# simonkosina/vbt

Measured on AMD Instinct MI355X. Metric: frames/sec end-to-end (detect+NMS+track), EfficientDet-Lite0 320x320, higher is better.
Workload: dtype int8

## Files before the change

vbt_amd/csrc/band_block.h:

```cpp
#pragma once
#include <type_traits>

#ifndef VBT_BD_WAVES
#define VBT_BD_WAVES 16
#endif
constexpr int BD_WAVES = VBT_BD_WAVES, BD_THREADS = 64 * BD_WAVES;
constexpr int BD_LIT = 3;
constexpr int BD_LIT_NODE = 1;
constexpr int BD_LIT_NODE_WIDE = 3;
constexpr int BD_WP_TAIL = 1024;

#ifdef VBT_BD_PROF
#define BD_STAMP(k) do { if (threadIdx.x == 0) a.prof[(long)blockIdx.x * 8 + (k)] = __builtin_amdgcn_s_memtime(); } while (0)
#else
#define BD_STAMP(k) do { } while (0)
#endif

struct BandArgs {
  const int8_t* x;
  int8_t* out;
  int H, W, Cout, rows, nbands;
  int C, CS;
  int NCG, KS;
  unsigned zx4;
  const v4i* wd;
  const int* bd;
  const float* md;
  Rq rqd;
  const v4i* wp;
  const int* bp;
  const float* mp;
  Rq rqp;
  int n_src, chain;
  const int8_t* src[3];
  int sh[3], sw[3], smode[3], spt[3], spl[3];
  AddQ sumq, preq;
#ifdef VBT_BD_PROF
  unsigned long long* prof;
#endif
};

__device__ __forceinline__ unsigned band_source4(const BandArgs& a, int j, long b, int iy, int ix, int cd, bool up2) {
  const int C = a.C;
  const int8_t* sb = a.src[j] + b * (long)a.sh[j] * a.sw[j] * C + 4 * cd;
  if (a.smode[j] == 0) return *(const unsigned*)(sb + (iy * a.sw[j] + ix) * C);
  if (a.smode[j] == 1) {
    int yy, xx;
    if (up2) { yy = iy >> 1; xx = ix >> 1; }
    else { yy = (iy * a.sh[j]) / a.H; xx = (ix * a.sw[j]) / a.W; }
    return *(const unsigned*)(sb + (yy * a.sw[j] + xx) * C);
  }
  unsigned lo = 0u, hi = 0u;
#pragma unroll
  for (int ky = 0; ky < 3; ky++) {
    const int yy = iy * 2 + ky - a.spt[j], yc = min(max(yy, 0), a.sh[j] - 1);
#pragma unroll
    for (int kx = 0; kx < 3; kx++) {
      const int xx = ix * 2 + kx - a.spl[j], xc = min(max(xx, 0), a.sw[j] - 1);
      unsigned t = *(const unsigned*)(sb + (yc * a.sw[j] + xc) * C);
      t = (yy == yc && xx == xc) ? (t ^ 0x80808080u) : 0u;
      lo = pk_max_u16(lo, t & 0x00FF00FFu);
      hi = pk_max_u16(hi, (t >> 8) & 0x00FF00FFu);
// ... 4 lines not shown

__device__ __forceinline__ uint4 band_source16(const BandArgs& a, int j, long b, int iy, int ix, int sg, bool up2) {
  const int C = a.C;
  const int8_t* sb = a.src[j] + b * (long)a.sh[j] * a.sw[j] * C + 16 * sg;
  if (a.smode[j] == 0) return *(const uint4*)(sb + (iy * a.sw[j] + ix) * C);
  if (a.smode[j] == 1) {
    int yy, xx;
    if (up2) { yy = iy >> 1; xx = ix >> 1; }
    else { yy = (iy * a.sh[j]) / a.H; xx = (ix * a.sw[j]) / a.W; }
    return *(const uint4*)(sb + (yy * a.sw[j] + xx) * C);
  }
  unsigned lo[4] = {0u, 0u, 0u, 0u}, hi[4] = {0u, 0u, 0u, 0u};
#pragma unroll
  for (int ky = 0; ky < 3; ky++) {
    const int yy = iy * 2 + ky - a.spt[j], yc = min(max(yy, 0), a.sh[j] - 1);
#pragma unroll
    for (int kx = 0; kx < 3; kx++) {
      const int xx = ix * 2 + kx - a.spl[j], xc = min(max(xx, 0), a.sw[j] - 1);
      const uint4 t4 = *(const uint4*)(sb + (yc * a.sw[j] + xc) * C);
      const bool in = yy == yc && xx == xc;
      const unsigned tt[4] = {t4.x, t4.y, t4.z, t4.w};
#pragma unroll
      for (int d = 0; d < 4; d++) {
        const unsigned t = in ? (tt[d] ^ 0x80808080u) : 0u;
        lo[d] = pk_max_u16(lo[d], t & 0x00FF00FFu);
        hi[d] = pk_max_u16(hi[d], (t >> 8) & 0x00FF00FFu);
      }
    }
  }
  return make_uint4((lo[0] | (hi[0] << 8)) ^ 0x80808080u, (lo[1] | (hi[1] << 8)) ^ 0x80808080u, (lo[2] | (hi[2] << 8)) ^ 0x80808080u,
                    (lo[3] | (hi[3] << 8)) ^ 0x80808080u);
}

template <int NW, int CT, bool NODES = true>
__device__ __forceinline__ void sepconv_band_body(const BandArgs& a, int local, unsigned char* bd_smem) {
  constexpr int nwaves = NW, nthreads = 64 * NW;
  constexpr bool C64 = CT == 64, CK = CT != 0;
  constexpr int CS_T = CT == 64 ? 80 : CT;
  static_assert(CT == 0 || CT == 64 || CT == 112, "compile-time widths: 64, 112");
  const long b = fdiv_small(local, frcp(a.nbands));
  const int band = local - (int)b * a.nbands;
  const int tid = threadIdx.x, wave = tid >> 6, lane = tid & 63, r = lane & 15, g = lane >> 4;
  const int y0 = band * a.rows, nr = min(a.rows, a.H - y0);
  const int PW = a.W + 2, NPh = (nr + 2) * PW, NPo = nr * a.W, NPG = (NPo + 15) >> 4;
  const int C = CK ? CT : a.C, CS = CK ? CS_T : a.CS;
  unsigned char* T0 = bd_smem;
  unsigned char* D = T0 + (a.rows + 2) * PW * CS;
  unsigned char* WP = D + (((a.rows * a.W + 15) >> 4) << 4) * CS;
  const int NT = (a.Cout + 15) >> 4, KS = CK ? (CT + 63) / 64 : a.KS, NCG = CK ? (CT + 15) / 16 : a.NCG;
  unsigned char* WB = WP + NT * KS * 1024;
  BD_STAMP(0);

  for (int i = tid; i < NT * KS * 64; i += nthreads) *(v4i*)(WP + 16 * i) = a.wp[i];
  if (tid < 4 * NT) *(uint4*)(WB + 16 * tid) = *(const uint4*)((const unsigned char*)a.bp + 16 * tid);
  else if (tid >= 32 && tid < 32 + 4 * NT) *(uint4*)(WB + 512 + 16 * (tid - 32)) = *(const uint4*)((const unsigned char*)a.mp + 16 * (tid - 32));
  const float rcp_pw = frcp(PW);
  if (NODES && a.n_src > 0) {
    const bool up2[3] = {a.H == 2 * a.sh[0] && a.W == 2 * a.sw[0], a.H == 2 * a.sh[1] && a.W == 2 * a.sw[1], a.H == 2 * a.sh[2] && a.W == 2 * a.sw[2]};
    if (CK || (C & 15) == 0) {
      constexpr int LITN = C64 ? BD_LIT_NODE : BD_LIT_NODE_WIDE;
      const int npp = C64 ? 4 : CS >> 4, nreal = C64 ? 4 : C >> 4;
      const float rcp_npp = frcp(npp);
      const int total = NPh * npp;
      for (int i0 = tid; i0 < total; i0 += LITN * nthreads) {
        uint4 us[LITN][3];
        int pofs[LITN];
#pragma unroll
        for (int k = 0; k < LITN; k++) {
          const int i = i0 + k * nthreads, ic = min(i, total - 1);
          const int p = C64 ? ic >> 2 : (CK ? ic / (CS_T >> 4) : fdiv_small(ic, rcp_npp)), sg = ic - p * npp;
          const int hy = fdiv_small(p, rcp_pw), hx = p - hy * PW;
          const int iy = y0 + hy - 1, ix = hx - 1;
          const bool in = i < total && sg < nreal && iy >= 0 && iy < a.H && ix >= 0 && ix < a.W;
          pofs[k] = i < total ? (p * CS + 16 * sg) | (in ? 0 : (1 << 30)) : -1;
#pragma unroll
          for (int j = 0; j < 3; j++) {
            us[k][j] = make_uint4(0u, 0u, 0u, 0u);
            if (j < a.n_src && in) us[k][j] = band_source16(a, j, b, iy, ix, sg, up2[j]);
          }
        }
#pragma unroll
        for (int k = 0; k < LITN; k++) {
          if (pofs[k] < 0) continue;
          uint4 v = make_uint4(a.zx4, a.zx4, a.zx4, a.zx4);
          if (!(pofs[k] >> 30)) {
            const unsigned u0[4] = {us[k][0].x, us[k][0].y, us[k][0].z, us[k][0].w}, u1[4] = {us[k][1].x, us[k][1].y, us[k][1].z, us[k][1].w},
// ... 64 lines not shown
      const int total = NPh * npp;
      for (int i0 = tid; i0 < total; i0 += BD_LIT * nthreads) {
        uint4 v[BD_LIT];
        int pofs[BD_LIT];
#pragma unroll
        for (int k = 0; k < BD_LIT; k++) {
          const int i = i0 + k * nthreads, ic = min(i, total - 1);
          const int p = CK ? ic / (CS_T >> 4) : fdiv_small(ic, rcp_npp), sg = ic - p * npp;
          const int hy = fdiv_small(p, rcp_pw), hx = p - hy * PW;
          const int iy = y0 + hy - 1, ix = hx - 1;
          pofs[k] = i < total ? p * CS + 16 * sg : -1;
          v[k] = z4;
          if (i < total && sg < nreal && iy >= 0 && iy < a.H && ix >= 0 && ix < a.W) v[k] = *(const uint4*)(xb + (iy * a.W + ix) * C + 16 * sg);
        }
#pragma unroll
        for (int k = 0; k < BD_LIT; k++)
          if (pofs[k] >= 0) *(uint4*)(T0 + pofs[k]) = v[k];
      }
    } else {
    const int ngp = CS >> 3, ng = C >> 3;
    const float rcp_ngp = frcp(ngp);
    const uint2 z2 = make_uint2(a.zx4, a.zx4);
    for (int i = tid; i < NPh * ngp; i += nthreads) {
      const int p = fdiv_small(i, rcp_ngp), sg = i - p * ngp;
      const int hy = fdiv_small(p, rcp_pw), hx = p - hy * PW;
      const int iy = y0 + hy - 1, ix = hx - 1;
      uint2 v = z2;
      if (sg < ng && iy >= 0 && iy < a.H && ix >= 0 && ix < a.W) v = *(const uint2*)(xb + (iy * a.W + ix) * C + 8 * sg);
      *(uint2*)(T0 + p * CS + 8 * sg) = v;
    }
    }
    }
  }
  const int cg = wave % NCG, sub = wave / NCG, nsub = nwaves / NCG;
  v4i wdv[3];
#pragma unroll
  for (int m = 0; m < 3; m++) wdv[m] = a.wd[(cg * 3 + m) * 64 + lane];
  const int4 bq = *(const int4*)(a.bd + 16 * cg + 4 * g);
  const float4 mu = *(const float4*)(a.md + 16 * cg + 4 * g);
  int tapoff[3];
#pragma unroll
  for (int m = 0; m < 3; m++) {
    const int tap = min(4 * m + g, 8);
    tapoff[m] = ((tap / 3) * PW + (tap % 3)) * CS;
  }
  const float rcp_w = frcp(a.W);
  __syncthreads();
  BD_STAMP(1);
  if (sub < nsub) {
    auto d_units = [&](auto full_c, auto u_c, int pg0) {
      constexpr int U = decltype(u_c)::value, FULL = decltype(full_c)::value;
      const unsigned char* pb[U];
      int slot[U];
#pragma unroll
      for (int u = 0; u < U; u++) {
        slot[u] = (pg0 + u * nsub) * 16 + r;
        const int sc = min(slot[u], NPo - 1);
        const int py = fdiv_small(sc, rcp_w);
        pb[u] = T0 + (sc + 2 * py) * CS + 16 * cg;
      }
      v4i bv[U][3], acc[U];
#pragma unroll
      for (int u = 0; u < U; u++)
#pragma unroll
        for (int m = 0; m < 3; m++) bv[u][m] = *(const v4i*)(pb[u] + tapoff[m]);
#pragma unroll
      for (int u = 0; u < U; u++) acc[u] = v4i_from(int4_plus(bq, FULL >= 2 ? RQ_KBIAS : 0));
#pragma unroll
      for (int m = 0; m < 3; m++)
#pragma unroll
        for (int u = 0; u < U; u++) acc[u] = __builtin_amdgcn_mfma_i32_16x16x64_i8(wdv[m], bv[u][m], acc[u], 0, 0, 0);
#pragma unroll
      for (int u = 0; u < U; u++) *(unsigned*)(D + slot[u] * CS + 16 * cg + 4 * g) = rq_pack_b<FULL>(acc[u], mu, a.rqd);
    };
    auto d_walk = [&](auto full_c) {
      int pg = sub;
      for (; pg + nsub < NPG; pg += 2 * nsub) d_units(full_c, std::integral_constant<int, 2>{}, pg);
      if (pg < NPG) d_units(full_c, std::integral_constant<int, 1>{}, pg);
    };
// ... 85 lines not shown
}

#ifndef VBT_BD_HEAD_WAVES
#define VBT_BD_HEAD_WAVES 8
#endif
#ifndef VBT_BD_HEAD_MAXPX
#define VBT_BD_HEAD_MAXPX 240
#endif
constexpr int BD_HEAD_WAVES = VBT_BD_HEAD_WAVES, BD_HEAD_MAXPX = VBT_BD_HEAD_MAXPX;
constexpr int BD_HEAD_WAVES_WIDE = 16;
#ifdef VBT_DEFINE_BAND_KERNELS
__device__ __forceinline__ int band_problem(const MultiTiles& mt) {
  int pi = 0;
#pragma unroll
  for (int i = 1; i < 12; i++)
    if (i < mt.n && (int)blockIdx.x >= mt.start[i]) pi = i;
  return pi;
}
__global__ __launch_bounds__(64 * BD_HEAD_WAVES) void sepconv_band_kernel(const BandArgs* __restrict__ probs, MultiTiles mt) {
  extern __shared__ __attribute__((aligned(16))) unsigned char bd_smem_dyn[];
  const int pi = band_problem(mt);
  sepconv_band_body<BD_HEAD_WAVES, 64, false>(probs[pi], (int)blockIdx.x - mt.start[pi], bd_smem_dyn);
}
__global__ __launch_bounds__(64 * BD_HEAD_WAVES_WIDE, 2) void sepconv_band_wide_kernel(const BandArgs* __restrict__ probs, MultiTiles mt) {
  extern __shared__ __attribute__((aligned(16))) unsigned char bd_smem_dyn[];
  const int pi = band_problem(mt);
  sepconv_band_body<BD_HEAD_WAVES_WIDE, 0, false>(probs[pi], (int)blockIdx.x - mt.start[pi], bd_smem_dyn);
}
__global__ __launch_bounds__(64 * BD_HEAD_WAVES_WIDE, 2) void sepconv_band_c112_kernel(const BandArgs* __restrict__ probs, MultiTiles mt) {
  extern __shared__ __attribute__((aligned(16))) unsigned char bd_smem_dyn[];
  const int pi = band_problem(mt);
  sepconv_band_body<BD_HEAD_WAVES_WIDE, 112, false>(probs[pi], (int)blockIdx.x - mt.start[pi], bd_smem_dyn);
}
__global__ __launch_bounds__(BD_THREADS) void sepconv_band_one_kernel(BandArgs a) {
  extern __shared__ __attribute__((aligned(16))) unsigned char bd_smem_dyn[];
  sepconv_band_body<BD_WAVES, 64>(a, (int)blockIdx.x, bd_smem_dyn);
}
__global__ __launch_bounds__(BD_THREADS) void sepconv_band_one_wide_kernel(BandArgs a) {
  extern __shared__ __attribute__((aligned(16))) unsigned char bd_smem_dyn[];
  sepconv_band_body<BD_WAVES, 0>(a, (int)blockIdx.x, bd_smem_dyn);
}
__global__ __launch_bounds__(BD_THREADS) void sepconv_band_one_c112_kernel(BandArgs a) {
  extern __shared__ __attribute__((aligned(16))) unsigned char bd_smem_dyn[];
  sepconv_band_body<BD_WAVES, 112>(a, (int)blockIdx.x, bd_smem_dyn);
}
#endif
```

vbt_amd/csrc/detector.hip:

```cpp
#include <algorithm>
#include <cmath>
#include <chrono>
#include <functional>
#include <map>
#include <set>
#include <type_traits>
#include <tuple>

#include "launchers.h"

namespace vbt {

static thread_local char g_err[512] = "";
void set_error(const char* fmt, ...) {
  va_list ap;
  va_start(ap, fmt);
  vsnprintf(g_err, sizeof(g_err), fmt, ap);
  va_end(ap);
}

bool lds_opt_in(const void* fn, LdsOptIn* state) {
  int dev = 0;
  if (hipGetDevice(&dev) != hipSuccess || dev < 0 || dev >= 64) { set_error("lds_opt_in: no current HIP device"); return false; }
  if (state->dev[dev] > 0) return true;
// ... 376 lines not shown
  if (xd_force != -100 && (xd_force < 100 || (s.xd2_ok && (xd_force < 200 ? s.xd2_gpw > 0 : s.xd2_gpw16 > 0)))) variant = std::min(xd_force, xd_force / 100 * 100 + s.xd.nchunks);
  ExpDwLaunch L;
  if (s.xd2_ok && (variant >= 100 || variant < 0)) {
    if (variant >= 200 && s.xd2_gpw16 == 0) { L.refuse(VBT_ERR_ARG, "expand + depthwise: plan asks for the 16-wave form on a step that does not support it"); return L; }
    if (variant >= 100 && variant < 200 && s.xd2_gpw == 0) { L.refuse(VBT_ERR_ARG, "expand + depthwise: plan asks for the 8-wave form on a step that does not support it"); return L; }
    const ExpDw2Args& a = s.xd2;
    L.second = true;
    L.nw = (variant >= 200 || (variant < 0 && s.xd2_gpw16 > 0)) ? 16 : 8;
    L.gpw = L.nw == 16 ? s.xd2_gpw16 : s.xd2_gpw;
    L.cpw = std::min(variant >= 100 ? variant % 100 : std::max(1, (a.nchunks * a.nbands * B + 1023) / 1024), a.nchunks);
    L.grid = (unsigned)(B * ((a.nchunks + L.cpw - 1) / L.cpw) * a.nbands);
    L.lds = s.xd2_lds;
    return L;
  }
  if (variant >= 100) { L.refuse(VBT_ERR_ARG, "expand + depthwise: plan asks for the second kernel form on a step that does not support it"); return L; }
  const ExpDwArgs& a = s.xd;
  L.cpw = variant > 0 ? variant : std::max(1, (a.nchunks * a.nbands * B + 511) / 512);
  L.grid = (unsigned)(B * ((a.nchunks + L.cpw - 1) / L.cpw) * a.nbands);
  L.lds = s.lds_bytes;
  return L;
}
static int launch_expdw_step(const vbt_model* m, const Step& s, int B, hipStream_t st, const int8_t* x, int8_t* out) {
  const ExpDwLaunch L = resolve_expdw(m, s, s.variant, B);
  if (L.rc) return L.report();
  const OpRec& dop = m->ops[s.d_op];
  if (L.second) {
    ExpDw2Args a = s.xd2;
    a.x = x; a.out = out; a.cpw = L.cpw;
    return launch_expdw2(a, dop.k, dop.stride, (a.Cin + 63) / 64, L.nw, L.gpw, L.grid, L.lds, st);
  }
  ExpDwArgs a = s.xd;
  a.x = x; a.out = out; a.cpw = L.cpw;
  return launch_expdw(a, dop.k, dop.stride, (a.Cin + 63) / 64, L.grid, L.lds, st);
}

static int launch_step(vbt_model* m, const Step& s, int B, hipStream_t st, const uint8_t* frames, float* boxes, float* scores,
                       float* classes, int* counts, int boff = 0) {
  if (m->pool_dirty) { const int rc = flush_uploads(m); if (rc) return rc; }
  const OpRec& op = m->ops[s.op];
  const TensorRec& to = m->tensors[op.output];
  auto TP = [&](int t) { return m->tptr[t] + (size_t)boff * m->telems[t]; };
  const uint8_t* frame0 = frames;
  int8_t* out = TP(op.output);
  auto member_tiles = [&](auto tiles_of) {
    MultiTiles mt;
    mt.n = (int)s.members.size();
    mt.start[0] = 0;
    for (int i = 0; i < mt.n; i++) mt.start[i + 1] = mt.start[i] + B * tiles_of(s.members[i]);
    return mt;
  };
  const Epi e{s.bias, s.mult, to.zero_point, op.act_min, op.act_max, make_rq(to.zero_point, op.act_min, op.act_max)};
  switch (s.family) {
    case F_STEM: {
      const TensorRec& ti = m->tensors[op.inputs[0]];
      long M = (long)B * to.h * to.w;
      dim3 grid((unsigned)((M + 63) / 64));
      stem_kernel<<<grid, 256, 0, st>>>(frame0, s.wp, e, out, M, ti.h, ti.w, to.h, to.w, to.c, op.pad_t, op.pad_l, ti.zero_point);
      return VBT_OK;
    }
    case F_PW: {
      if (s.members.empty())
        return launch_pw_step(m, s, B, st, TP(m->ops[s.res_op >= 0 ? s.p_op : s.op].inputs[0]),
                              s.res_op >= 0 ? TP(m->ops[s.res_op].inputs[1]) : nullptr, out);
      if (boff != 0) { set_error("merged pointwise convs: sub-batch streams are not supported (VBT_SUBSTREAMS)"); return VBT_ERR_ARG; }
      PwMulti pm;
      memset(&pm, 0, sizeof(pm));
// ... 44 lines not shown
    }
    case F_RESIZE: {
      const TensorRec& ti = m->tensors[op.inputs[0]];
      long total = (long)B * to.h * to.w * (to.c / 4);
      resize_kernel<<<dim3((unsigned)((total + 255) / 256)), 256, 0, st>>>(TP(op.inputs[0]), out, total, ti.h, ti.w, ti.c,
                                                                            to.h, to.w);
      return VBT_OK;
    }
    case F_MULTI: {
      if (boff != 0) {
        for (const Step& ms : s.members) {
          Step t = ms;
          t.variant = s.variant;
          const int rc = launch_step(m, t, B, st, frames, boxes, scores, classes, counts, boff);
          if (rc) return rc;
        }
        return VBT_OK;
      }
      const MultiTiles mt = member_tiles([](const Step& ms) { return ms.fa.tiles_x * ms.fa.tiles_y; });
      const OpRec& dop = m->ops[s.d_op];
      return launch_fused_multi(s.d_multi, mt, dop.k, dop.stride, s.nbp, s.variant != 0, s.lds_bytes, (unsigned)mt.start[mt.n], st);
    }
    case F_MBCONV:
    case F_NODE:
    case F_SEPCONV: {
      FusedArgs a = s.fa;
      a.x = s.e_op >= 0 ? TP(m->ops[s.e_op].inputs[0]) : TP(m->ops[s.d_op].inputs[0]);
      for (int j = 0; j < 3; j++) a.src[j] = s.src_tensor[j] >= 0 ? TP(s.src_tensor[j]) : nullptr;
      a.out = out;
      return launch_fused_step(m, s, a, B, st);
    }
    case F_BAND: {
      if (boff != 0) { set_error("fused_sepconv_band: sub-batch streams are not supported (VBT_SUBSTREAMS)"); return VBT_ERR_ARG; }
      if (s.members.empty()) return launch_band_one(s.bd_args, (unsigned)(B * s.band_tiles), s.lds_bytes, st);
      const MultiTiles mt = member_tiles([](const Step& ms) { return ms.band_tiles; });
      return launch_band_multi(s.d_band, mt, s.members[0].bd_args.C, (unsigned)mt.start[mt.n], s.lds_bytes, st);
    }
    case F_EXPDW:
      return launch_expdw_step(m, s, B, st, TP(m->ops[s.e_op].inputs[0]), out);
    case F_STEMBLK: {
      StemBlockArgs a = s.sb;
      a.frames = frame0;
      a.out = out;
      return launch_stem_block(a, a.rqs.full && a.rqd.full && a.rqp.full, (unsigned)((long)B * a.tiles_x * a.tiles_y), st);
    }
    case F_POST: {
      PostArgs p;
      int base = 0;
      p.C = m->hdr.num_classes > 0 ? m->hdr.num_classes : 1;
      for (int l = 0; l < 5; l++) {
        const TensorRec& tc = m->tensors[op.inputs[l]];
        p.cls[l] = TP(op.inputs[l]);
        p.box[l] = TP(op.inputs[5 + l]);
        p.base[l] = base;
        base += tc.h * tc.w * tc.c / p.C;
      }
      p.base[5] = base;
      p.anchors = m->d_anchors;
      p.tables = m->d_luts;
      p.A = m->hdr.num_anchors;
      p.max_det = m->hdr.max_detections;
      p.iou_thr = m->hdr.nms_iou_threshold;
      int qmin = 128;
      for (int q = 127; q >= -128; q--)
        if (m->post_tables_host[q + 128] >= m->hdr.nms_score_threshold) qmin = q; else break;
      p.qmin = qmin;
      const int lds = post_lds_bytes(p.A);
      if (lds > 64 * 1024) VBT_LDS_OPT_IN(postprocess_kernel);
      if (lds > 160 * 1024 || p.A > 65535) { set_error("decode + NMS: %d anchors do not fit the kernel (LDS %d bytes, 16-bit anchor index)", p.A, lds); return VBT_ERR_CAPACITY; }
// ... 17 lines not shown
  hipEvent_t e0, e1;
  if (hipEventCreate(&e0) != hipSuccess || hipEventCreate(&e1) != hipSuccess) return 1e30;
  float ms = 1e30f;
  int rc = VBT_OK;
  if (nconc <= 1) {
    rc = launch_step(m, s, B, nullptr, m->frames_stage, m->out_boxes, m->out_scores, m->out_classes, m->out_counts);
    (void)hipEventRecord(e0, nullptr);
    for (int r = 0; r < reps && !rc; r++)
      rc = launch_step(m, s, B, nullptr, m->frames_stage, m->out_boxes, m->out_scores, m->out_classes, m->out_counts);
    (void)hipEventRecord(e1, nullptr);
    if (hipEventSynchronize(e1) != hipSuccess || hipEventElapsedTime(&ms, e0, e1) != hipSuccess) ms = 1e30f;
    ms /= reps;
  } else {
    (void)hipDeviceSynchronize();
    for (int i = 0; i < nconc && !rc; i++)
      rc = launch_step(m, s, B, cs[i], m->frames_stage, m->out_boxes, m->out_scores, m->out_classes, m->out_counts);
    (void)hipDeviceSynchronize();
    auto t0 = std::chrono::steady_clock::now();
    for (int r = 0; r < reps; r++)
      for (int i = 0; i < nconc && !rc; i++)
        rc = launch_step(m, s, B, cs[i], m->frames_stage, m->out_boxes, m->out_scores, m->out_classes, m->out_counts);
    (void)hipDeviceSynchronize();
    ms = (float)(std::chrono::duration<double, std::milli>(std::chrono::steady_clock::now() - t0).count() / (reps * nconc));
  }
  (void)hipEventDestroy(e0);
  (void)hipEventDestroy(e1);
  return rc ? 1e30 : ms;
}

static bool is_fused_tile(int family) { return family == F_MBCONV || family == F_SEPCONV || family == F_NODE; }
static bool variant_ok(const vbt_model* m, const Step& st, int v) {
  if (st.family == F_PW) return !st.members.empty() || !resolve_pw(m, st, v, m->max_batch).rc;
  if (is_fused_tile(st.family)) return !resolve_fused(m, st, v, m->max_batch).rc;
  return st.family != F_EXPDW || !resolve_expdw(m, st, v, m->max_batch).rc;
}

static std::vector<int> candidate_variants(const vbt_model* m, const Step& st) {
  std::vector<int> cand{-1};
  const OpRec& op = m->ops[st.op];
  if (st.family == F_DW) {
    cand = {0};
    for (int r : {1, 2, 4, 8, 16})
      if (r <= m->tensors[op.output].h) cand.push_back(r);
    if (m->tensors[op.output].c % 8 == 0) { cand.push_back(100); cand.push_back(101); }
  } else if (st.family == F_PW && st.KS64 <= 4) {
    cand = {0, 1};
  } else if (st.family == F_PW) {
    cand = {-1, 2, 3, 4, 5, 6};
  } else if (is_fused_tile(st.family)) {
    cand = {0, 1, 3, 5};
    if (st.family == F_MBCONV && st.fa.nch3 > 0 && st.nbp <= 2 && st.fa.KSe >= 1 && st.fa.KSe <= 4) { cand.push_back(9); cand.push_back(11); }
    if (st.family == F_MBCONV && st.nbp <= 2 && (st.fa.KSe == 1 || st.fa.KSe == 2)) {
      cand.push_back(17);
      if (st.fa.nch3 > 0) cand.push_back(25);
    }
  } else if (st.family == F_MULTI) {
    cand = {0, 1};
  } else if (st.family == F_EXPDW) {
    cand.clear();
    for (int cpw : {1, 2, 3, 4, 6})
      if (cpw <= st.xd.nchunks) cand.push_back(cpw);
    if (st.xd2_ok)
      for (int cpw : {1, 2, 3, 4, 6})
        if (cpw <= st.xd.nchunks) {
          if (st.xd2_gpw > 0) cand.push_back(100 + cpw);
          if (st.xd2_gpw16 > 0) cand.push_back(200 + cpw);
        }
  }
  cand.erase(std::remove_if(cand.begin(), cand.end(), [&](int v) { return !variant_ok(m, st, v); }), cand.end());
  return cand;
}

static void autotune(vbt_model* m) {
  const int B = (m->max_batch + m->n_sub - 1) / m->n_sub, reps = 4;
  for (Group& g : m->groups) {
    bool single = g.alts.size() == 1 && g.alts[0].steps.size() == 1;
    if (single) {
      int f = g.alts[0].steps[0].family;
      if (f != F_DW && f != F_PW) continue;
    }
    for (Alt& a : g.alts) {
      a.ms = 0;
      for (Step& st : a.steps) {
        const std::vector<int> cand = candidate_variants(m, st);
        double best = 1e30;
        int bestv = -1;
        for (int v : cand) {
          Step t = st;
          t.variant = v;
          double ms = time_step(m, t, B, reps);
          if (getenv("VBT_AUTOTUNE_VERBOSE") && cand.size() > 1 && atoi(getenv("VBT_AUTOTUNE_VERBOSE")) > 1)
            fprintf(stderr, "[autotune]   op %d %s v%d %.1fus\n", st.op, kFamilyName[st.family], v, ms * 1e3);
          if (ms < best) { best = ms; bestv = v; }
        }
        st.variant = bestv;
        st.tuned_ms = best;
        a.ms += best;
      }
    }
    int bi = 0;
// ... 675 lines not shown
```

vbt_amd/csrc/k_band.hip:

```cpp
#define VBT_DEFINE_BAND_KERNELS 1
#include "launchers.h"

namespace vbt {

static int band_attrs() {
  VBT_LDS_OPT_IN(sepconv_band_kernel);
  VBT_LDS_OPT_IN(sepconv_band_one_kernel);
  VBT_LDS_OPT_IN(sepconv_band_wide_kernel);
  VBT_LDS_OPT_IN(sepconv_band_one_wide_kernel);
  VBT_LDS_OPT_IN(sepconv_band_c112_kernel);
  VBT_LDS_OPT_IN(sepconv_band_one_c112_kernel);
  return VBT_OK;
}

int launch_band_one(const BandArgs& a, unsigned grid, int lds_bytes, hipStream_t st) {
  if (band_attrs()) return VBT_ERR_HIP;
  static const bool generic = getenv("VBT_BAND_GENERIC") != nullptr;
  if (a.C == 64) sepconv_band_one_kernel<<<dim3(grid), BD_THREADS, lds_bytes, st>>>(a);
  else if (a.C == 112 && a.CS == 112 && !generic) sepconv_band_one_c112_kernel<<<dim3(grid), BD_THREADS, lds_bytes, st>>>(a);
  else sepconv_band_one_wide_kernel<<<dim3(grid), BD_THREADS, lds_bytes, st>>>(a);
  return VBT_OK;
}

int launch_band_multi(const BandArgs* d_probs, const MultiTiles& mt, int C, unsigned grid, int lds_bytes, hipStream_t st) {
  if (band_attrs()) return VBT_ERR_HIP;
  static const bool generic = getenv("VBT_BAND_GENERIC") != nullptr;
  if (C == 64) sepconv_band_kernel<<<dim3(grid), 64 * BD_HEAD_WAVES, lds_bytes, st>>>(d_probs, mt);
  else if (C == 112 && !generic) sepconv_band_c112_kernel<<<dim3(grid), 64 * BD_HEAD_WAVES_WIDE, lds_bytes, st>>>(d_probs, mt);
  else sepconv_band_wide_kernel<<<dim3(grid), 64 * BD_HEAD_WAVES_WIDE, lds_bytes, st>>>(d_probs, mt);
  return VBT_OK;
}

int launch_expdw(const ExpDwArgs& a, int k, int stride, int KS64, unsigned grid_x, int lds_bytes, hipStream_t st) {
  const dim3 grid(grid_x);
#define XD_LAUNCH(KK, S)                                                                                             \
  do {                                                                                                               \
    VBT_LDS_OPT_IN(expdw_image_kernel<KK, S, 2>);                                                                    \
    VBT_LDS_OPT_IN(expdw_image_kernel<KK, S, 3>);                                                                    \
    VBT_LDS_OPT_IN(expdw_image_kernel<KK, S, 4>);                                                                    \
    if (KS64 == 2) expdw_image_kernel<KK, S, 2><<<grid, XD_THREADS, lds_bytes, st>>>(a);                             \
    else if (KS64 == 3) expdw_image_kernel<KK, S, 3><<<grid, XD_THREADS, lds_bytes, st>>>(a);                        \
    else expdw_image_kernel<KK, S, 4><<<grid, XD_THREADS, lds_bytes, st>>>(a);                                       \
  } while (0)
  if (k == 3 && stride == 1) XD_LAUNCH(3, 1);
  else if (k == 5 && stride == 1) XD_LAUNCH(5, 1);
  else XD_LAUNCH(5, 2);
#undef XD_LAUNCH
  return VBT_OK;
}

template <int KK, int S, int KS64, int NW, int GPW>
static int launch_expdw2_t(const ExpDw2Args& a, unsigned grid, int lds_bytes, hipStream_t st) {
  VBT_LDS_OPT_IN(expdw2_kernel<KK, S, KS64, NW, GPW>);
  expdw2_kernel<KK, S, KS64, NW, GPW><<<dim3(grid), 64 * NW, lds_bytes, st>>>(a);
  return VBT_OK;
}

int launch_expdw2(const ExpDw2Args& a, int k, int stride, int KS64, int nw, int gpw, unsigned grid, int lds_bytes, hipStream_t st) {
#define XD2_GPW(KK, KS)                                                                    \
  do {                                                                                     \
// ... 41 lines not shown
```

vbt_amd/csrc/launchers.h:

```cpp
#pragma once
#include "dev_common.h"

namespace vbt {
#include "fused_block.h"
#include "stem_block.h"
#include "image_block.h"
#include "expdw_block.h"
#include "expdw2_block.h"
#include "band_block.h"

struct FusedLaunch {
  int k, stride, nbp;
  bool expand;
  bool mdw;
  bool nt3;
  bool ppw2;
  bool dw64;
  int lds_bytes;
  unsigned grid;
};
int launch_fused_block(const FusedArgs& a, const FusedLaunch& L, hipStream_t st);
int launch_fused_multi(const FusedArgs* d_args, const MultiTiles& mt, int k, int stride, int nbp, bool mdw, int lds_bytes, unsigned grid,
                       hipStream_t st);
int launch_dw_tile(const DwTileArgs& a, int k, int stride, bool mdw, dim3 grid, int lds_bytes, hipStream_t st);
int launch_mbconv_image(const FusedArgs& a, const ImageBundle& wb, int k, int stride, int maxu, int PW, int PH, int NB, int lds_bytes, int B,
                        hipStream_t st);
int launch_band_one(const BandArgs& a, unsigned grid, int lds_bytes, hipStream_t st);
int launch_band_multi(const BandArgs* d_probs, const MultiTiles& mt, int C, unsigned grid, int lds_bytes, hipStream_t st);
int launch_expdw(const ExpDwArgs& a, int k, int stride, int KS64, unsigned grid, int lds_bytes, hipStream_t st);
int launch_expdw2(const ExpDw2Args& a, int k, int stride, int KS64, int nw, int gpw, unsigned grid, int lds_bytes, hipStream_t st);
int launch_stem_block(const StemBlockArgs& a, bool full_range, unsigned grid, hipStream_t st);

}
```

vbt_amd/csrc/planner.h:

```cpp
#pragma once

static int conv_kb(const vbt_model* m, const OpRec& op) {
  const bool off = getenv("VBT_NO_KBIAS") != nullptr;
  if (off || (op.type != OP_STEM && op.type != OP_PW && op.type != OP_DW)) return 0;
  const TensorRec& tin = m->tensors[op.inputs[0]];
  const TensorRec& tout = m->tensors[op.output];
  const int8_t* w = (const int8_t*)(m->blob.data() + op.w_off);
  const int32_t* bq = (const int32_t*)(m->blob.data() + op.b_off);
  const bool dw = op.type == OP_DW;
  const int N = tout.c, K = dw ? op.k * op.k : op.k * op.k * tin.c;
  for (int co = 0; co < N; co++) {
    long long sa = 0;
    for (int k = 0; k < K; k++) sa += std::abs((int)(dw ? w[(size_t)k * N + co] : w[(size_t)co * K + k]));
    if (255 * sa + std::llabs((long long)bq[co]) >= (1ll << 22) - 1) return 0;
  }
  return 1;
}

static void choose_tile(int OH, int OW, int KK, int S, bool expand, int* TXo, int* TYo, int slots = 64) {
  double best = 1e300;
  for (int TX = 1; TX <= std::min(OW, 64); TX++) {
    int TXp = (TX + 3) & ~3;
    int TY = std::min(OH, slots / TXp);
    if (TY < 1) continue;
// ... 162 lines not shown
    std::vector<v4i> wp3;
    pack_weights64(wpj, tout.c, Ce, nch3, s.nbp, wp3, &kmap);
    long *d1, *d2;
    v4i* d3;
    if ((rc = upload(m, pack_expand48(we, Ce, tin.c, a.KSe), &d1)) || (rc = upload(m, pack_dw_diag(wd, Ce, kk, 48), &d2)) || (rc = upload(m, wp3, &d3))) return rc;
    a.we3 = d1; a.wdm3 = d2; a.wp3 = d3; a.nch3 = nch3; a.KSp3 = nch3;
  }
  if (expand && tin.h * tin.w <= 400 && tout.h * tout.w <= 400 && (rc = make_image_bundle(m, e_op, d_op, p_op, a.KSe, &s.ib))) return rc;
  *out = s;
  return VBT_OK;
}

static const Alt* tile_alt(const Group& g, int family) {
  for (int i = (int)g.alts.size() - 1; i >= 0; i--)
    if (g.alts[i].steps.size() == 1 && g.alts[i].steps[0].family == family) return &g.alts[i];
  return nullptr;
}
static const Alt* band_alt(const Group& g) {
  for (int i = (int)g.alts.size() - 1; i >= 0; i--)
    if (g.alts[i].steps.size() == 1 && g.alts[i].steps[0].family == F_BAND && g.alts[i].steps[0].members.empty()) return &g.alts[i];
  return nullptr;
}

static bool band_ok(const vbt_model* m, int d_op, int p_op) {
  if (m->flags & VBT_MODEL_NO_BAND) return false;
  if (const char* ns = getenv("VBT_SUBSTREAMS")) if (atoi(ns) > 1) return false;
  const OpRec& d = m->ops[d_op];
  const OpRec& p = m->ops[p_op];
  const TensorRec& ti = m->tensors[d.inputs[0]];
  const TensorRec& to = m->tensors[p.output];
  return d.k == 3 && d.stride == 1 && d.pad_t == 1 && d.pad_l == 1 && ti.c % 8 == 0 && ti.c >= 16 && ti.c <= 128 && to.c <= 128 && to.h == ti.h &&
         to.w == ti.w && ti.w <= 160;
}
static int band_lds(const BandArgs& a) {
  const int NT = (a.Cout + 15) / 16;
  return (a.rows + 2) * (a.W + 2) * a.CS + (((a.rows * a.W + 15) >> 4) << 4) * a.CS + NT * a.KS * 1024 + BD_WP_TAIL;
}
static int make_band(vbt_model* m, int d_op, int p_op, int sum_op, const NodeSrc* ns, Step* out) {
  const OpRec& dop = m->ops[d_op];
  const OpRec& pop = m->ops[p_op];
  const TensorRec& tin = m->tensors[dop.inputs[0]];
  const TensorRec& td = m->tensors[dop.output];
  const TensorRec& to = m->tensors[pop.output];
  Step s;
  s.family = F_BAND;
  s.op = p_op;
  s.d_op = d_op;
  s.p_op = p_op;
  s.sum_op = sum_op;
  BandArgs& a = s.bd_args;
  memset(&a, 0, sizeof(a));
  a.H = tin.h; a.W = tin.w; a.Cout = to.c;
  const int C = tin.c;
  a.C = C;
  a.CS = ((C + 15) / 16 | 1) * 16;
  a.NCG = (C + 15) / 16;
  a.KS = (C + 63) / 64;
  static const int band_px_env = getenv("VBT_BAND_PX") ? atoi(getenv("VBT_BAND_PX")) : 0;
  const int band_px = band_px_env > 0 ? band_px_env : (m->max_batch <= 8 ? 64 : 320);
  const int nb = std::max(1, (tin.h * tin.w + band_px - 1) / band_px);
  a.rows = (tin.h + nb - 1) / nb;
  a.nbands = (tin.h + a.rows - 1) / a.rows;
  a.zx4 = (unsigned)(tin.zero_point & 255) * 0x01010101u;
  const int8_t* wd = (const int8_t*)(m->blob.data() + dop.w_off);
  v4i *dpd, *dpp;
  int* dbd;
  float* dmd;
  int rc;
  if ((rc = upload(m, pack_band_dw(wd, C), &dpd)) || (rc = upload(m, pack_band_pw((const int8_t*)(m->blob.data() + pop.w_off), to.c, C), &dpp)) ||
      (rc = upload(m, fold_bias((const int32_t*)(m->blob.data() + dop.b_off), wd, C, 9, tin.zero_point, W_TAPS, a.NCG * 16), &dbd)) ||
      (rc = upload(m, pad_floats((const float*)(m->blob.data() + dop.m_off), C, a.NCG * 16), &dmd)))
    return rc;
  a.wd = dpd; a.wp = dpp; a.bd = dbd; a.md = dmd;
  a.bp = m->op_steps[p_op].bias;
  a.mp = m->op_steps[p_op].mult;
  a.rqd = make_rq(td.zero_point, dop.act_min, dop.act_max, conv_kb(m, dop));
  a.rqp = make_rq(to.zero_point, pop.act_min, pop.act_max, conv_kb(m, pop));
  a.x = m->tptr[dop.inputs[0]];
  a.out = m->tptr[pop.output];
  if (sum_op >= 0) {
    fill_node_sources(a, *ns, m, sum_op);
    a.x = nullptr;
    for (int j = 0; j < ns->n; j++) a.src[j] = m->tptr[ns->tensor[j]];
  }
  s.band_tiles = a.nbands;
  s.lds_bytes = band_lds(a);
  std::vector<BandArgs> one{a};
  if ((rc = upload(m, one, &s.d_band))) return rc;
  s.cost = cost_of(m, {d_op, p_op, sum_op}, ns);
  *out = s;
  return VBT_OK;
}

static int batch_heads(vbt_model* m) {
  struct Info { int gi, chain, depth; };
  std::vector<Info> heads;
  std::map<int, std::pair<int, int>> by_tensor;
  int nchains = 0, first = -1;
  for (int gi = 0; gi < (int)m->groups.size(); gi++) {
    const Group& g = m->groups[gi];
    const Alt* fap = tile_alt(g, F_SEPCONV);
    if (!fap) continue;
    const Step& st = fap->steps[0];
    if (m->ops[st.d_op].level < 0) continue;
    int tin = m->ops[st.d_op].inputs[0], tout = m->ops[st.p_op].output;
    auto it = by_tensor.find(tin);
// ... 848 lines not shown
```

vbt_amd/csrc/weight_pack.h:

```cpp
#pragma once

static void pack_weights(const int8_t* w, int N, int K, int KS, int NB, const std::vector<int>* kmap, std::vector<long>& out) {
  out.assign((size_t)NB * KS * 4 * 64, 0);
  int8_t* o = (int8_t*)out.data();
  for (int nb = 0; nb < NB; nb++)
    for (int ks = 0; ks < KS; ks++)
      for (int t = 0; t < 4; t++)
        for (int lane = 0; lane < 64; lane++) {
          int i = lane & 15, g = lane >> 4;
          int co = 64 * nb + 16 * (i >> 2) + 4 * t + (i & 3);
          for (int j = 0; j < 8; j++) {
            int kp = 32 * ks + 8 * g + j;
            int k = kmap ? (kp < (int)kmap->size() ? (*kmap)[kp] : -1) : (kp < K ? kp : -1);
            int8_t v = (co < N && k >= 0) ? w[(size_t)co * K + k] : 0;
            o[((((size_t)(nb * KS + ks) * 4 + t) * 64 + lane) * 8) + j] = v;
          }
        }
}

static void pack_weights64(const int8_t* w, int N, int K, int KS, int NB, std::vector<v4i>& out, const std::vector<int>* kmap = nullptr) {
  out.assign((size_t)NB * KS * 4 * 64, (v4i){0, 0, 0, 0});
  int8_t* o = (int8_t*)out.data();
  for (int nb = 0; nb < NB; nb++)
    for (int ks = 0; ks < KS; ks++)
// ... 95 lines not shown
  std::vector<int> kmap((size_t)(Ce / 48) * 64, -1);
  for (int c = 0; c < Ce / 48; c++)
    for (int q = 0; q < 48; q++) kmap[(size_t)c * 64 + q] = 48 * c + q;
  return kmap;
}

static std::vector<v4i> pack_band_dw(const int8_t* w, int C) {
  const int NCG = (C + 15) / 16;
  std::vector<v4i> out((size_t)NCG * 3 * 64, (v4i){0, 0, 0, 0});
  int8_t* o = (int8_t*)out.data();
  for (int cg = 0; cg < NCG; cg++)
    for (int mi = 0; mi < 3; mi++)
      for (int lane = 0; lane < 64; lane++) {
        const int i = lane & 15, g = lane >> 4, ch = 16 * cg + i, tap = 4 * mi + g;
        for (int j = 0; j < 16; j++) o[(((size_t)(cg * 3 + mi) * 64 + lane) * 16) + j] = (tap < 9 && j == i && ch < C) ? w[(size_t)tap * C + ch] : 0;
      }
  return out;
}
static std::vector<v4i> pack_band_pw(const int8_t* w, int N, int C) {
  const int NT = (N + 15) / 16, KS = (C + 63) / 64;
  std::vector<v4i> out((size_t)NT * KS * 64, (v4i){0, 0, 0, 0});
  int8_t* o = (int8_t*)out.data();
  for (int t = 0; t < NT; t++)
    for (int ks = 0; ks < KS; ks++)
      for (int lane = 0; lane < 64; lane++) {
        const int i = lane & 15, g = lane >> 4, co = 16 * t + i;
        for (int j = 0; j < 16; j++) {
          const int k = 64 * ks + 16 * g + j;
          o[((((size_t)t * KS + ks) * 64 + lane) * 16) + j] = (co < N && k < C) ? w[(size_t)co * C + k] : 0;
        }
      }
  return out;
}

static std::vector<int> stem_kmap() {
  std::vector<int> kmap(32, -1);
  for (int g = 0; g < 3; g++)
    for (int j = 0; j < 8; j++) kmap[8 * g + j] = (g * 3 + j / 3) * 3 + j % 3;
  for (int j = 0; j < 3; j++) kmap[24 + j] = (j * 3 + 2) * 3 + 2;
  return kmap;
}
static std::vector<long> pack_stem_block_stem(const int8_t* w) {
  std::vector<long> out(2 * 64, 0);
  int8_t* o = (int8_t*)out.data();
  for (int t = 0; t < 2; t++)
    for (int lane = 0; lane < 64; lane++) {
      const int i = lane & 15, kg = lane >> 4, co = 8 * (i >> 2) + 4 * t + (i & 3);
      for (int j = 0; j < 8; j++) {
        const int f = kg < 3 ? kg * 9 + j : (j < 3 ? j * 9 + 8 : -1);
        o[((size_t)t * 64 + lane) * 8 + j] = f >= 0 ? w[(size_t)co * 27 + f] : 0;
      }
    }
  return out;
}
static std::vector<long> pack_stem_block_proj(const int8_t* w, int N) {
  std::vector<long> out(64, 0);
  int8_t* o = (int8_t*)out.data();
  for (int lane = 0; lane < 64; lane++) {
    const int i = lane & 15, kg = lane >> 4;
    for (int j = 0; j < 8; j++) o[(size_t)lane * 8 + j] = i < N ? w[(size_t)i * 32 + 8 * kg + j] : 0;
  }
  return out;
}

static std::vector<v4i> pack_expdw_expand(const int8_t* w, int Ce, int K) {
  const int nch = (Ce + 63) / 64, KS = (K + 63) / 64;
// ... 46 lines not shown
```

Before: 115,700.

## Add chained depthwise-to-pointwise band kernel keeping intermediate in registers

Adds a chained form of the 64-channel separable-conv band kernel. Each wave computes all four depthwise channel groups for its pixels and feeds the requantized result straight from registers into the pointwise MFMA, which removes the LDS staging buffer D and the sync between the two stages. Depthwise weights move into LDS, and the pointwise weights are repacked so the register layout matches. The planner picks this form by default when max_batch > 8, and a plan variant or env var can override it. The cost is more per-wave registers and redundant depthwise weight loads per pixel group.

```diff
diff --git a/vbt_amd/csrc/band_block.h b/vbt_amd/csrc/band_block.h
--- a/vbt_amd/csrc/band_block.h
+++ b/vbt_amd/csrc/band_block.h
@@ -9,6 +9,7 @@
 constexpr int BD_LIT_NODE = 1;
 constexpr int BD_LIT_NODE_WIDE = 3;
 constexpr int BD_WP_TAIL = 1024;
+constexpr int BD_WD_CHAIN = 12 * 1024 + 512;
 
 #ifdef VBT_BD_PROF
 #define BD_STAMP(k) do { if (threadIdx.x == 0) a.prof[(long)blockIdx.x * 8 + (k)] = __builtin_amdgcn_s_memtime(); } while (0)
@@ -28,6 +29,7 @@
   const float* md;
   Rq rqd;
   const v4i* wp;
+  const v4i* wpc;
   const int* bp;
   const float* mp;
   Rq rqp;
@@ -98,9 +100,10 @@
                     (lo[3] | (hi[3] << 8)) ^ 0x80808080u);
 }
 
-template <int NW, int CT, bool NODES = true>
+template <int NW, int CT, bool NODES = true, bool CHAIN = false>
 __device__ __forceinline__ void sepconv_band_body(const BandArgs& a, int local, unsigned char* bd_smem) {
   constexpr int nwaves = NW, nthreads = 64 * NW;
+  static_assert(!CHAIN || CT == 64, "the chained form is built for 64-channel maps");
   constexpr bool C64 = CT == 64, CK = CT != 0;
   constexpr int CS_T = CT == 64 ? 80 : CT;
   static_assert(CT == 0 || CT == 64 || CT == 112, "compile-time widths: 64, 112");
@@ -112,12 +115,18 @@
   const int C = CK ? CT : a.C, CS = CK ? CS_T : a.CS;
   unsigned char* T0 = bd_smem;
   unsigned char* D = T0 + (a.rows + 2) * PW * CS;
-  unsigned char* WP = D + (((a.rows * a.W + 15) >> 4) << 4) * CS;
+  unsigned char* WP = CHAIN ? D : D + (((a.rows * a.W + 15) >> 4) << 4) * CS;
   const int NT = (a.Cout + 15) >> 4, KS = CK ? (CT + 63) / 64 : a.KS, NCG = CK ? (CT + 15) / 16 : a.NCG;
   unsigned char* WB = WP + NT * KS * 1024;
   BD_STAMP(0);
 
-  for (int i = tid; i < NT * KS * 64; i += nthreads) *(v4i*)(WP + 16 * i) = a.wp[i];
+  const v4i* wpg = CHAIN ? a.wpc : a.wp;
+  for (int i = tid; i < NT * KS * 64; i += nthreads) *(v4i*)(WP + 16 * i) = wpg[i];
+  if constexpr (CHAIN) {
+    for (int i = tid; i < 12 * 64; i += nthreads) *(v4i*)(WB + BD_WP_TAIL + 16 * i) = a.wd[i];
+    if (tid >= 64 && tid < 80) *(uint4*)(WB + BD_WP_TAIL + 12 * 1024 + 16 * (tid - 64)) = *(const uint4*)((const unsigned char*)a.bd + 16 * (tid - 64));
+    else if (tid >= 96 && tid < 112) *(uint4*)(WB + BD_WP_TAIL + 12 * 1024 + 256 + 16 * (tid - 96)) = *(const uint4*)((const unsigned char*)a.md + 16 * (tid - 96));
+  }
   if (tid < 4 * NT) *(uint4*)(WB + 16 * tid) = *(const uint4*)((const unsigned char*)a.bp + 16 * tid);
   else if (tid >= 32 && tid < 32 + 4 * NT) *(uint4*)(WB + 512 + 16 * (tid - 32)) = *(const uint4*)((const unsigned char*)a.mp + 16 * (tid - 32));
   const float rcp_pw = frcp(PW);
@@ -248,19 +257,93 @@
     }
     }
   }
+  int tapoff[3];
+#pragma unroll
+  for (int m = 0; m < 3; m++) {
+    const int tap = min(4 * m + g, 8);
+    tapoff[m] = ((tap / 3) * PW + (tap % 3)) * CS;
+  }
+  const float rcp_w = frcp(a.W);
+  if constexpr (CHAIN) {
+    const unsigned char* WD = WB + BD_WP_TAIL;
+    const unsigned char* WDB = WD + 12 * 1024;
+    __syncthreads();
+    BD_STAMP(1);
+    int8_t* ob = a.out + ((b * a.H + y0) * (long)a.W) * a.Cout + 4 * g;
+    const bool dword_out = (a.Cout & 3) == 0;
+    auto chain = [&](auto fd_c, auto u_c, int pg0) {
+      constexpr int U = decltype(u_c)::value, FULL = decltype(fd_c)::value;
+      int slot[U];
+      const unsigned char* pb[U];
+#pragma unroll
+      for (int u = 0; u < U; u++) {
+        slot[u] = (pg0 + u * nwaves) * 16 + r;
+        const int sc = min(slot[u], NPo - 1);
+        const int py = fdiv_small(sc, rcp_w);
+        pb[u] = T0 + (sc + 2 * py) * CS;
+      }
+      v4i dv[U];
+      {
+#pragma unroll
+        for (int cg = 0; cg < 4; cg++) {
+          v4i wdv[3], bv[U][3], acc[U];
+#pragma unroll
+          for (int m = 0; m < 3; m++) wdv[m] = *(const v4i*)(WD + ((cg * 3 + m) * 64 + lane) * 16);
+          const int4 bq = *(const int4*)(WDB + 64 * cg + 16 * g);
+          const float4 mu = *(const float4*)(WDB + 256 + 64 * cg + 16 * g);
+#pragma unroll
+          for (int u = 0; u < U; u++)
+#pragma unroll
+            for (int m = 0; m < 3; m++) bv[u][m] = *(const v4i*)(pb[u] + tapoff[m] + 16 * cg);
+#pragma unroll
+          for (int u = 0; u < U; u++) acc[u] = v4i_from(int4_plus(bq, FULL >= 2 ? RQ_KBIAS : 0));
+#pragma unroll
+          for (int m = 0; m < 3; m++)
+#pragma unroll
+            for (int u = 0; u < U; u++) acc[u] = __builtin_amdgcn_mfma_i32_16x16x64_i8(wdv[m], bv[u][m], acc[u], 0, 0, 0);
+#pragma unroll
+          for (int u = 0; u < U; u++) dv[u][cg] = (int)rq_pack_b<FULL>(acc[u], mu, a.rqd);
+          __builtin_amdgcn_sched_barrier(0);
+        }
+      }
+      rq_dispatch(a.rqp, [&](auto fp_c) {
+        constexpr int FULL = decltype(fp_c)::value;
+        for (int t = 0; t < NT; t++) {
+          const int c0 = 16 * t + 4 * g;
+          const v4i wv = *(const v4i*)(WP + (t * 64 + lane) * 16);
+          const int4 bb = *(const int4*)(WB + 4 * c0);
+          const float4 mm = *(const float4*)(WB + 512 + 4 * c0);
+          v4i acc[U];
+#pragma unroll
+          for (int u = 0; u < U; u++) acc[u] = __builtin_amdgcn_mfma_i32_16x16x64_i8(wv, dv[u], v4i_from(int4_plus(bb, FULL >= 2 ? RQ_KBIAS : 0)), 0, 0, 0);
+#pragma unroll
+          for (int u = 0; u < U; u++) {
+            const unsigned d = rq_pack_b<FULL>(acc[u], mm, a.rqp);
+            if (slot[u] < NPo && c0 < a.Cout) {
+              int8_t* o = ob + (long)slot[u] * a.Cout + 16 * t;
+              if (dword_out) *(unsigned*)o = d;
+              else
+                for (int j = 0; j < 4; j++)
+                  if (c0 + j < a.Cout) o[j] = (int8_t)(d >> (8 * j));
+            }
+          }
+        }
+      });
+    };
+    rq_dispatch(a.rqd, [&](auto fd_c) {
+      int pg = wave;
+      for (; pg + nwaves < NPG; pg += 2 * nwaves) chain(fd_c, std::integral_constant<int, 2>{}, pg);
+      if (pg < NPG) chain(fd_c, std::integral_constant<int, 1>{}, pg);
+    });
+    BD_STAMP(3);
+    return;
+  }
   const int cg = wave % NCG, sub = wave / NCG, nsub = nwaves / NCG;
   v4i wdv[3];
 #pragma unroll
   for (int m = 0; m < 3; m++) wdv[m] = a.wd[(cg * 3 + m) * 64 + lane];
   const int4 bq = *(const int4*)(a.bd + 16 * cg + 4 * g);
   const float4 mu = *(const float4*)(a.md + 16 * cg + 4 * g);
-  int tapoff[3];
-#pragma unroll
-  for (int m = 0; m < 3; m++) {
-    const int tap = min(4 * m + g, 8);
-    tapoff[m] = ((tap / 3) * PW + (tap % 3)) * CS;
-  }
-  const float rcp_w = frcp(a.W);
   __syncthreads();
   BD_STAMP(1);
   if (sub < nsub) {
@@ -412,10 +495,19 @@
   const int pi = band_problem(mt);
   sepconv_band_body<BD_HEAD_WAVES_WIDE, 112, false>(probs[pi], (int)blockIdx.x - mt.start[pi], bd_smem_dyn);
 }
+__global__ __launch_bounds__(64 * BD_HEAD_WAVES) __attribute__((amdgpu_waves_per_eu(6))) void sepconv_band_chain_kernel(const BandArgs* __restrict__ probs, MultiTiles mt) {
+  extern __shared__ __attribute__((aligned(16))) unsigned char bd_smem_dyn[];
+  const int pi = band_problem(mt);
+  sepconv_band_body<BD_HEAD_WAVES, 64, false, true>(probs[pi], (int)blockIdx.x - mt.start[pi], bd_smem_dyn);
+}
 __global__ __launch_bounds__(BD_THREADS) void sepconv_band_one_kernel(BandArgs a) {
   extern __shared__ __attribute__((aligned(16))) unsigned char bd_smem_dyn[];
   sepconv_band_body<BD_WAVES, 64>(a, (int)blockIdx.x, bd_smem_dyn);
 }
+__global__ __launch_bounds__(BD_THREADS) void sepconv_band_one_chain_kernel(BandArgs a) {
+  extern __shared__ __attribute__((aligned(16))) unsigned char bd_smem_dyn[];
+  sepconv_band_body<BD_WAVES, 64, true, true>(a, (int)blockIdx.x, bd_smem_dyn);
+}
 __global__ __launch_bounds__(BD_THREADS) void sepconv_band_one_wide_kernel(BandArgs a) {
   extern __shared__ __attribute__((aligned(16))) unsigned char bd_smem_dyn[];
   sepconv_band_body<BD_WAVES, 0>(a, (int)blockIdx.x, bd_smem_dyn);
diff --git a/vbt_amd/csrc/detector.hip b/vbt_amd/csrc/detector.hip
--- a/vbt_amd/csrc/detector.hip
+++ b/vbt_amd/csrc/detector.hip
@@ -432,6 +432,27 @@
   ExpDwArgs a = s.xd;
   a.x = x; a.out = out; a.cpw = L.cpw;
   return launch_expdw(a, dop.k, dop.stride, (a.Cin + 63) / 64, L.grid, L.lds, st);
+}
+
+struct BandLaunch : Verdict { bool chained = false; int lds = 0; };
+static bool band_chainable(const Step& s) {
+  if (s.members.empty()) return s.bd_args.wpc != nullptr;
+  for (const Step& ms : s.members)
+    if (!ms.bd_args.wpc) return false;
+  return true;
+}
+static BandLaunch resolve_band(const vbt_model* m, const Step& s, int variant, int) {
+  BandLaunch L;
+  const bool can = band_chainable(s);
+  if (variant < -1 || variant > 1) { L.refuse(VBT_ERR_ARG, "fused_sepconv_band: no kernel form %d", variant); return L; }
+  if (variant == 1 && !can) { L.refuse(VBT_ERR_ARG, "fused_sepconv_band: plan asks for the chained form on a step that does not support it"); return L; }
+  static const int bd_force = getenv("VBT_BAND_VARIANT") ? atoi(getenv("VBT_BAND_VARIANT")) : -100;
+  if (bd_force == 0 || (bd_force == 1 && can)) variant = bd_force;
+  L.chained = variant == 1 || (variant < 0 && can && m->max_batch > 8);
+  if (s.members.empty()) L.lds = band_lds(s.bd_args, L.chained);
+  for (const Step& ms : s.members) L.lds = std::max(L.lds, band_lds(ms.bd_args, L.chained));
+  if (L.lds > 160 * 1024) L.refuse(VBT_ERR_ARG, "fused_sepconv_band: a band of %d bytes does not fit the LDS", L.lds);
+  return L;
 }
 
 static int launch_step(vbt_model* m, const Step& s, int B, hipStream_t st, const uint8_t* frames, float* boxes, float* scores,
@@ -542,9 +563,11 @@
     }
     case F_BAND: {
       if (boff != 0) { set_error("fused_sepconv_band: sub-batch streams are not supported (VBT_SUBSTREAMS)"); return VBT_ERR_ARG; }
-      if (s.members.empty()) return launch_band_one(s.bd_args, (unsigned)(B * s.band_tiles), s.lds_bytes, st);
+      const BandLaunch L = resolve_band(m, s, s.variant, B);
+      if (L.rc) return L.report();
+      if (s.members.empty()) return launch_band_one(s.bd_args, L.chained, (unsigned)(B * s.band_tiles), L.lds, st);
       const MultiTiles mt = member_tiles([](const Step& ms) { return ms.band_tiles; });
-      return launch_band_multi(s.d_band, mt, s.members[0].bd_args.C, (unsigned)mt.start[mt.n], s.lds_bytes, st);
+      return launch_band_multi(s.d_band, mt, s.members[0].bd_args.C, L.chained, (unsigned)mt.start[mt.n], L.lds, st);
     }
     case F_EXPDW:
       return launch_expdw_step(m, s, B, st, TP(m->ops[s.e_op].inputs[0]), out);
@@ -628,6 +651,7 @@
 static bool variant_ok(const vbt_model* m, const Step& st, int v) {
   if (st.family == F_PW) return !st.members.empty() || !resolve_pw(m, st, v, m->max_batch).rc;
   if (is_fused_tile(st.family)) return !resolve_fused(m, st, v, m->max_batch).rc;
+  if (st.family == F_BAND) return !resolve_band(m, st, v, m->max_batch).rc;
   return st.family != F_EXPDW || !resolve_expdw(m, st, v, m->max_batch).rc;
 }
 
@@ -662,6 +686,8 @@
           if (st.xd2_gpw > 0) cand.push_back(100 + cpw);
           if (st.xd2_gpw16 > 0) cand.push_back(200 + cpw);
         }
+  } else if (st.family == F_BAND) {
+    cand = {-1, 0, 1};
   }
   cand.erase(std::remove_if(cand.begin(), cand.end(), [&](int v) { return !variant_ok(m, st, v); }), cand.end());
   return cand;
diff --git a/vbt_amd/csrc/k_band.hip b/vbt_amd/csrc/k_band.hip
--- a/vbt_amd/csrc/k_band.hip
+++ b/vbt_amd/csrc/k_band.hip
@@ -6,6 +6,8 @@
 static int band_attrs() {
   VBT_LDS_OPT_IN(sepconv_band_kernel);
   VBT_LDS_OPT_IN(sepconv_band_one_kernel);
+  VBT_LDS_OPT_IN(sepconv_band_chain_kernel);
+  VBT_LDS_OPT_IN(sepconv_band_one_chain_kernel);
   VBT_LDS_OPT_IN(sepconv_band_wide_kernel);
   VBT_LDS_OPT_IN(sepconv_band_one_wide_kernel);
   VBT_LDS_OPT_IN(sepconv_band_c112_kernel);
@@ -13,19 +15,23 @@
   return VBT_OK;
 }
 
-int launch_band_one(const BandArgs& a, unsigned grid, int lds_bytes, hipStream_t st) {
+int launch_band_one(const BandArgs& a, bool chained, unsigned grid, int lds_bytes, hipStream_t st) {
   if (band_attrs()) return VBT_ERR_HIP;
   static const bool generic = getenv("VBT_BAND_GENERIC") != nullptr;
-  if (a.C == 64) sepconv_band_one_kernel<<<dim3(grid), BD_THREADS, lds_bytes, st>>>(a);
+  if (chained && (a.C != 64 || !a.wpc)) { set_error("fused_sepconv_band: the chained form needs a 64-channel map"); return VBT_ERR_ARG; }
+  if (chained) sepconv_band_one_chain_kernel<<<dim3(grid), BD_THREADS, lds_bytes, st>>>(a);
+  else if (a.C == 64) sepconv_band_one_kernel<<<dim3(grid), BD_THREADS, lds_bytes, st>>>(a);
   else if (a.C == 112 && a.CS == 112 && !generic) sepconv_band_one_c112_kernel<<<dim3(grid), BD_THREADS, lds_bytes, st>>>(a);
   else sepconv_band_one_wide_kernel<<<dim3(grid), BD_THREADS, lds_bytes, st>>>(a);
   return VBT_OK;
 }
 
-int launch_band_multi(const BandArgs* d_probs, const MultiTiles& mt, int C, unsigned grid, int lds_bytes, hipStream_t st) {
+int launch_band_multi(const BandArgs* d_probs, const MultiTiles& mt, int C, bool chained, unsigned grid, int lds_bytes, hipStream_t st) {
   if (band_attrs()) return VBT_ERR_HIP;
   static const bool generic = getenv("VBT_BAND_GENERIC") != nullptr;
-  if (C == 64) sepconv_band_kernel<<<dim3(grid), 64 * BD_HEAD_WAVES, lds_bytes, st>>>(d_probs, mt);
+  if (chained && C != 64) { set_error("fused_sepconv_band: the chained form needs 64-channel maps"); return VBT_ERR_ARG; }
+  if (chained) sepconv_band_chain_kernel<<<dim3(grid), 64 * BD_HEAD_WAVES, lds_bytes, st>>>(d_probs, mt);
+  else if (C == 64) sepconv_band_kernel<<<dim3(grid), 64 * BD_HEAD_WAVES, lds_bytes, st>>>(d_probs, mt);
   else if (C == 112 && !generic) sepconv_band_c112_kernel<<<dim3(grid), 64 * BD_HEAD_WAVES_WIDE, lds_bytes, st>>>(d_probs, mt);
   else sepconv_band_wide_kernel<<<dim3(grid), 64 * BD_HEAD_WAVES_WIDE, lds_bytes, st>>>(d_probs, mt);
   return VBT_OK;
diff --git a/vbt_amd/csrc/launchers.h b/vbt_amd/csrc/launchers.h
--- a/vbt_amd/csrc/launchers.h
+++ b/vbt_amd/csrc/launchers.h
@@ -25,8 +25,8 @@
 int launch_dw_tile(const DwTileArgs& a, int k, int stride, bool mdw, dim3 grid, int lds_bytes, hipStream_t st);
 int launch_mbconv_image(const FusedArgs& a, const ImageBundle& wb, int k, int stride, int maxu, int PW, int PH, int NB, int lds_bytes, int B,
                         hipStream_t st);
-int launch_band_one(const BandArgs& a, unsigned grid, int lds_bytes, hipStream_t st);
-int launch_band_multi(const BandArgs* d_probs, const MultiTiles& mt, int C, unsigned grid, int lds_bytes, hipStream_t st);
+int launch_band_one(const BandArgs& a, bool chained, unsigned grid, int lds_bytes, hipStream_t st);
+int launch_band_multi(const BandArgs* d_probs, const MultiTiles& mt, int C, bool chained, unsigned grid, int lds_bytes, hipStream_t st);
 int launch_expdw(const ExpDwArgs& a, int k, int stride, int KS64, unsigned grid, int lds_bytes, hipStream_t st);
 int launch_expdw2(const ExpDw2Args& a, int k, int stride, int KS64, int nw, int gpw, unsigned grid, int lds_bytes, hipStream_t st);
 int launch_stem_block(const StemBlockArgs& a, bool full_range, unsigned grid, hipStream_t st);
diff --git a/vbt_amd/csrc/planner.h b/vbt_amd/csrc/planner.h
--- a/vbt_amd/csrc/planner.h
+++ b/vbt_amd/csrc/planner.h
@@ -218,9 +218,10 @@
   return d.k == 3 && d.stride == 1 && d.pad_t == 1 && d.pad_l == 1 && ti.c % 8 == 0 && ti.c >= 16 && ti.c <= 128 && to.c <= 128 && to.h == ti.h &&
          to.w == ti.w && ti.w <= 160;
 }
-static int band_lds(const BandArgs& a) {
+static int band_lds(const BandArgs& a, bool chained = false) {
   const int NT = (a.Cout + 15) / 16;
-  return (a.rows + 2) * (a.W + 2) * a.CS + (((a.rows * a.W + 15) >> 4) << 4) * a.CS + NT * a.KS * 1024 + BD_WP_TAIL;
+  const int t0 = (a.rows + 2) * (a.W + 2) * a.CS, wp = NT * a.KS * 1024 + BD_WP_TAIL;
+  return chained ? t0 + wp + BD_WD_CHAIN : t0 + (((a.rows * a.W + 15) >> 4) << 4) * a.CS + wp;
 }
 static int make_band(vbt_model* m, int d_op, int p_op, int sum_op, const NodeSrc* ns, Step* out) {
   const OpRec& dop = m->ops[d_op];
@@ -249,7 +250,7 @@
   a.nbands = (tin.h + a.rows - 1) / a.rows;
   a.zx4 = (unsigned)(tin.zero_point & 255) * 0x01010101u;
   const int8_t* wd = (const int8_t*)(m->blob.data() + dop.w_off);
-  v4i *dpd, *dpp;
+  v4i *dpd, *dpp, *dpc = nullptr;
   int* dbd;
   float* dmd;
   int rc;
@@ -257,7 +258,8 @@
       (rc = upload(m, fold_bias((const int32_t*)(m->blob.data() + dop.b_off), wd, C, 9, tin.zero_point, W_TAPS, a.NCG * 16), &dbd)) ||
       (rc = upload(m, pad_floats((const float*)(m->blob.data() + dop.m_off), C, a.NCG * 16), &dmd)))
     return rc;
-  a.wd = dpd; a.wp = dpp; a.bd = dbd; a.md = dmd;
+  if (C == 64 && to.c <= 64 && (rc = upload(m, pack_band_pw_chain((const int8_t*)(m->blob.data() + pop.w_off), to.c, C), &dpc))) return rc;
+  a.wd = dpd; a.wp = dpp; a.wpc = dpc; a.bd = dbd; a.md = dmd;
   a.bp = m->op_steps[p_op].bias;
   a.mp = m->op_steps[p_op].mult;
   a.rqd = make_rq(td.zero_point, dop.act_min, dop.act_max, conv_kb(m, dop));
diff --git a/vbt_amd/csrc/weight_pack.h b/vbt_amd/csrc/weight_pack.h
--- a/vbt_amd/csrc/weight_pack.h
+++ b/vbt_amd/csrc/weight_pack.h
@@ -151,6 +151,21 @@
       }
   return out;
 }
+static std::vector<v4i> pack_band_pw_chain(const int8_t* w, int N, int C) {
+  const int NT = (N + 15) / 16;
+  std::vector<v4i> out((size_t)NT * 64, (v4i){0, 0, 0, 0});
+  int8_t* o = (int8_t*)out.data();
+  for (int t = 0; t < NT; t++)
+    for (int lane = 0; lane < 64; lane++) {
+      const int i = lane & 15, g = lane >> 4, co = 16 * t + i;
+      for (int cg = 0; cg < 4; cg++)
+        for (int j = 0; j < 4; j++) {
+          const int k = 16 * cg + 4 * g + j;
+          o[((size_t)t * 64 + lane) * 16 + 4 * cg + j] = (co < N && k < C) ? w[(size_t)co * C + k] : 0;
+        }
+    }
+  return out;
+}
 
 static std::vector<int> stem_kmap() {
   std::vector<int> kmap(32, -1);
```

Measured after the change: 118,000 (median of 6 runs). 1.02x the previous value.
